# liortalker/MindTheEdge

Hardware: AMD Instinct MI355X
Metric: training images/sec, PackNet-SAN+edge-loss 384x1280 bf16 (higher is better)
Workload: dtype bf16; 1 GPU; T8: PackNet-SAN + silog + 4-scale depth-edge loss training step, 384x1280, 8 frames/GPU, dropout 0.5, flip 0.5; global_batch=8, height=384, width=1280, parallelism=single GPU

## Files before the change

mindtheedge_amd/csrc/heads_misc.hip:

```cpp
#include "common.hpp"
#include <atomic>

int tap_wgrad_mfma_launch(const bf16_t* x, long ldx, const float* m, float* rec, long rec_stride, int B, int H, int W, int C, int sgn, int up2, int has_db,
                          int max_wgs, int* groups, hipStream_t st);
namespace {

template <typename T> __device__ __forceinline__ void ld8(const T* p, float* v);
template <> __device__ __forceinline__ void ld8<bf16_t>(const bf16_t* p, float* v) { unpack16<bf16_t>(*(const u32x4_t*)p, v); }
template <> __device__ __forceinline__ void ld8<float>(const float* p, float* v) {
    unpack16<float>(*(const u32x4_t*)p, v); unpack16<float>(*(const u32x4_t*)(p + 4), v + 4);
}
template <typename T> __device__ __forceinline__ void st8(T* p, const float* v);
template <> __device__ __forceinline__ void st8<bf16_t>(bf16_t* p, const float* v) { *(u32x4_t*)p = pack16<bf16_t>(v); }
template <> __device__ __forceinline__ void st8<float>(float* p, const float* v) {
    *(u32x4_t*)p = pack16<float>(v); *(u32x4_t*)(p + 4) = pack16<float>(v + 4);
}

struct HeadArgs {
    const void* x; long ldx;
    const float* w; const float* bias;
    float* out;
    const float* dlogit;
    void* dx; long lddx;
    float* dw;
// ... 482 lines not shown
#pragma unroll
        for (int r = 0; r < 3; ++r) { const int yy = yl - 1 + r; iok[r] = (unsigned)yy < (unsigned)h; ir[r] = inv + ((long)b * h + min(max(yy, 0), h - 1)) * wl; }
        float uw[3][3];
#pragma unroll
        for (int k = 0; k < 3; ++k) {
            const int xx = x0 - 1 + k; const bool ok = (unsigned)xx < (unsigned)wl; const int xc = min(max(xx, 0), wl - 1);
#pragma unroll
            for (int r = 0; r < 3; ++r) uw[r][k] = (ok && iok[r]) ? ir[r][xc] : 0.f;
        }
        const int x1 = min(x0 + SEG, wl);
        for (int x = x0; x < x1; ++x) {
            u32x4_t raw[4];
#pragma unroll
            for (int q = 0; q < 4; ++q) raw[q] = *(const u32x4_t*)(base + ((long)(q >> 1) * W + 2 * x + (q & 1)) * lddy);
#pragma unroll
            for (int q = 0; q < 4; ++q) {
                float g[P];
                unpack16<T>(raw[q], g);
                const int qy = q >> 1, qx = q & 1;
#pragma unroll
                for (int ky = 0; ky < 3; ++ky)
#pragma unroll
                    for (int kx = 0; kx < 3; ++kx) {
                        const float uu = uw[(qy + ky + 1) >> 1][(qx + kx + 1) >> 1];
#pragma unroll
                        for (int e = 0; e < P; ++e) dacc[ky * 3 + kx][e] = fmaf(g[e], uu, dacc[ky * 3 + kx][e]);
                    }
            }
            if (x + 1 < x1) {
                const int xx = x + 2; const bool ok = xx < wl; const int xc = min(xx, wl - 1);
#pragma unroll
                for (int r = 0; r < 3; ++r) { uw[r][0] = uw[r][1]; uw[r][1] = uw[r][2]; uw[r][2] = (ok && iok[r]) ? ir[r][xc] : 0.f; }
            }
        }
    }
    const int lane = threadIdx.x & 63, wave = threadIdx.x >> 6;
#pragma unroll
    for (int tp = 0; tp < 9; ++tp)
#pragma unroll
        for (int e = 0; e < P; ++e) {
            float v = dacc[tp][e];
            for (int off = cpr; off < 64; off <<= 1) v += __shfl_xor(v, off, 64);
            if (lane < cpr) sred[wave * (N * 9) + (lane * P + e) * 9 + tp] = v;
        }
    __syncthreads();
    for (int i = threadIdx.x; i < N * 9; i += blockDim.x)
        records[(long)blockIdx.x * (N * 9) + i] = (sred[i] + sred[N * 9 + i]) + (sred[2 * N * 9 + i] + sred[3 * N * 9 + i]);
}
__global__ __launch_bounds__(256) void rank1_wgrad_reduce_kernel(const float* __restrict__ records, int nrec, int N, float* __restrict__ dst, long dst_stride) {
    const int i = blockIdx.x * 4 + (threadIdx.x >> 6), lane = threadIdx.x & 63;
    if (i >= N * 9) return;
    float s = 0.f;
    for (int r = lane; r < nrec; r += 64) s += records[(long)r * (N * 9) + i];
    for (int off = 32; off > 0; off >>= 1) s += __shfl_xor(s, off, 64);
    if (lane == 0) dst[(long)(i / 9) * dst_stride + i % 9] = s;
}

__global__ void upsample2_f32_kernel(const float* __restrict__ inv, float* __restrict__ out, int B, int h, int w) {
    const long n = (long)B * 4 * h * w;
    for (long i = blockIdx.x * (long)blockDim.x + threadIdx.x; i < n; i += (long)gridDim.x * blockDim.x) {
        const int X = (int)(i % (2 * w)); const long t = i / (2 * w); const int Y = (int)(t % (2 * h)); const int b = (int)(t / (2 * h));
        out[i] = inv[((long)b * h + (Y >> 1)) * w + (X >> 1)];
    }
}

template <typename T>
__global__ void copy_channels_kernel(const T* __restrict__ src, long lds_, T* __restrict__ dst, long ldd, long npix, int C) {
    constexpr int P = Elem<T>::PER16;
    const int cpr = C / P;
    const long n = npix * cpr;
    for (long i = blockIdx.x * (long)blockDim.x + threadIdx.x; i < n; i += (long)gridDim.x * blockDim.x) {
        const long pix = i / cpr; const int cc = (int)(i % cpr);
        *(u32x4_t*)(dst + pix * ldd + cc * P) = *(const u32x4_t*)(src + pix * lds_ + cc * P);
    }
}

__global__ void split_record_kernel(const float* __restrict__ src, float* __restrict__ d0, int n0, float* __restrict__ d1, int n1) {
    for (int i = blockIdx.x * blockDim.x + threadIdx.x; i < n0 + n1; i += gridDim.x * blockDim.x) {
        const float v = src[i];
        if (i < n0) d0[i] = v; else d1[i - n0] = v;
    }
}

template <typename T>
__global__ void add_channels_kernel(const T* __restrict__ a, long lda, const T* __restrict__ b, long ldb, T* __restrict__ out, long ldo,
                                    long npix, int C) {
    constexpr int P = Elem<T>::PER16;
    const int cpr = C / P;
    const long n = npix * cpr;
    for (long i = blockIdx.x * (long)blockDim.x + threadIdx.x; i < n; i += (long)gridDim.x * blockDim.x) {
        const long pix = i / cpr; const int cc = (int)(i % cpr);
        float va[P], vb[P];
        unpack16<T>(*(const u32x4_t*)(a + pix * lda + cc * P), va);
        unpack16<T>(*(const u32x4_t*)(b + pix * ldb + cc * P), vb);
#pragma unroll
        for (int k = 0; k < P; ++k) va[k] += vb[k];
        *(u32x4_t*)(out + pix * ldo + cc * P) = pack16<T>(va);
    }
}

__global__ void adam_kernel(float* __restrict__ p, const float* __restrict__ g, float* __restrict__ m, float* __restrict__ v,
                            long n, float lr, float b1, float b2, float eps, float bc1, float bc2s, float gscale) {
    const long n4 = n >> 2;
    for (long i = blockIdx.x * (long)blockDim.x + threadIdx.x; i < n4; i += (long)gridDim.x * blockDim.x) {
        f32x4_t pp = ((f32x4_t*)p)[i], gg = ((const f32x4_t*)g)[i], mm = ((f32x4_t*)m)[i], vv = ((f32x4_t*)v)[i];
#pragma unroll
        for (int k = 0; k < 4; ++k) {
            const float gk = gg[k] * gscale;
            mm[k] = b1 * mm[k] + (1.f - b1) * gk;
            vv[k] = b2 * vv[k] + (1.f - b2) * gk * gk;
            const float denom = sqrtf(vv[k]) / bc2s + eps;
            pp[k] -= (lr / bc1) * (mm[k] / denom);
        }
        ((f32x4_t*)p)[i] = pp; ((f32x4_t*)m)[i] = mm; ((f32x4_t*)v)[i] = vv;
    }
    if (blockIdx.x == 0 && threadIdx.x < (n & 3)) {
        const long i = (n4 << 2) + threadIdx.x;
        const float gk = g[i] * gscale;
        const float mk = b1 * m[i] + (1.f - b1) * gk, vk = b2 * v[i] + (1.f - b2) * gk * gk;
        m[i] = mk; v[i] = vk;
        p[i] -= (lr / bc1) * (mk / (sqrtf(vk) / bc2s + eps));
    }
}

__global__ void adam_dev_kernel(float* __restrict__ p, const float* __restrict__ g, float* __restrict__ m, float* __restrict__ v,
                                long n, const float* __restrict__ hyper, float b1, float b2, float eps, float gscale) {
    const float lr = hyper[0], bc1 = hyper[1], bc2s = hyper[2];
    const long n4 = n >> 2;
    for (long i = blockIdx.x * (long)blockDim.x + threadIdx.x; i < n4; i += (long)gridDim.x * blockDim.x) {
        f32x4_t pp = ((f32x4_t*)p)[i], gg = ((const f32x4_t*)g)[i], mm = ((f32x4_t*)m)[i], vv = ((f32x4_t*)v)[i];
#pragma unroll
        for (int k = 0; k < 4; ++k) {
            const float gk = gg[k] * gscale;
            mm[k] = b1 * mm[k] + (1.f - b1) * gk;
            vv[k] = b2 * vv[k] + (1.f - b2) * gk * gk;
            const float denom = sqrtf(vv[k]) / bc2s + eps;
            pp[k] -= (lr / bc1) * (mm[k] / denom);
        }
        ((f32x4_t*)p)[i] = pp; ((f32x4_t*)m)[i] = mm; ((f32x4_t*)v)[i] = vv;
    }
    if (blockIdx.x == 0 && threadIdx.x < (n & 3)) {
        const long i = (n4 << 2) + threadIdx.x;
        const float gk = g[i] * gscale;
        const float mk = b1 * m[i] + (1.f - b1) * gk, vk = b2 * v[i] + (1.f - b2) * gk * gk;
        m[i] = mk; v[i] = vk;
        p[i] -= (lr / bc1) * (mk / (sqrtf(vk) / bc2s + eps));
    }
}

__device__ __forceinline__ void bilin_src(int dst, int in, float scale, int& i0, int& i1, float& l1) {
    float src = scale * ((float)dst + 0.5f) - 0.5f;
    if (src < 0.f) src = 0.f;
    i0 = (int)src; if (i0 > in - 1) i0 = in - 1;
    i1 = i0 < in - 1 ? i0 + 1 : i0;
    l1 = src - (float)i0;
}
__global__ void resize_bilinear_kernel(const float* __restrict__ x, float* __restrict__ y, float* __restrict__ dx, const float* __restrict__ dy,
                                       int B, int h, int w, int H, int W) {
    const float sh = (float)h / (float)H, sw = (float)w / (float)W;
    const long n = (long)B * H * W;
    for (long i = blockIdx.x * (long)blockDim.x + threadIdx.x; i < n; i += (long)gridDim.x * blockDim.x) {
        const int X = (int)(i % W), Y = (int)((i / W) % H), b = (int)(i / ((long)W * H));
        int y0, y1, x0, x1; float ly, lx;
        bilin_src(Y, h, sh, y0, y1, ly); bilin_src(X, w, sw, x0, x1, lx);
        const long base = (long)b * h * w;
        const float w00 = (1.f - ly) * (1.f - lx), w01 = (1.f - ly) * lx, w10 = ly * (1.f - lx), w11 = ly * lx;
        if (y) {
            y[i] = w00 * x[base + (long)y0 * w + x0] + w01 * x[base + (long)y0 * w + x1] + w10 * x[base + (long)y1 * w + x0] + w11 * x[base + (long)y1 * w + x1];
        } else {
            const float g = dy[i];
            atomicAdd(dx + base + (long)y0 * w + x0, w00 * g); atomicAdd(dx + base + (long)y0 * w + x1, w01 * g);
            atomicAdd(dx + base + (long)y1 * w + x0, w10 * g); atomicAdd(dx + base + (long)y1 * w + x1, w11 * g);
        }
    }
}

inline int stream_grid(long n, int per = 256) { long g = (n + per - 1) / per; return (int)(g > 8192 ? 8192 : (g < 1 ? 1 : g)); }
int g_head_mfma = 1;
inline bool head_ok(int C) { const int cb = C >> 3; return C % 8 == 0 && cb >= 1 && cb <= 64 && (cb & (cb - 1)) == 0; }
inline long head_strips(int B, int H, int W, int C) {
    const int pxw = 256 / (C >> 3);
    return (long)((W + pxw - 1) / pxw) * ((H + HEAD_ROWS - 1) / HEAD_ROWS) * B;
}
template <typename F> int head_resident(F f, size_t lds, std::atomic<int>* cache) {
    int v = cache->load(std::memory_order_relaxed);
    if (v == 0) {
        int per_cu = 0, dev = 0, cus = 256;
        if (hipOccupancyMaxActiveBlocksPerMultiprocessor(&per_cu, f, 256, lds) != hipSuccess || per_cu < 1) per_cu = 2;
        hipDeviceProp_t prop;
        if (hipGetDevice(&dev) == hipSuccess && hipGetDeviceProperties(&prop, dev) == hipSuccess && prop.multiProcessorCount > 0) cus = prop.multiProcessorCount;
        v = per_cu * cus;
        cache->store(v, std::memory_order_relaxed);
    }
    return v;
}
inline long head_record_stride(int C) { return ((long)C * 9 + 1 + 3) / 4 * 4; }
constexpr int HEAD_WGRAD_MAX_BLOCKS = 1024;

}

#ifdef MTE_DEV
extern "C" int mtei_set_head_mfma(int v) { g_head_mfma = v; return MTE_OK; }
#endif

extern "C" {

int mte_invdepth_fwd(const void* x, long ldx, const float* w, const float* bias, float* out,
                     int B, int H, int W, int C, float min_depth, int dtype, hipStream_t stream) {
    (void)hipGetLastError();
    if (!x || !w || !bias || !out || !head_ok(C)) return MTE_ERR_ARG;
    HeadArgs a{}; a.x = x; a.ldx = ldx; a.w = w; a.bias = bias; a.out = out; a.B = B; a.H = H; a.W = W; a.C = C;
    a.inv_min_depth = 1.f / min_depth; a.npix = (long)B * H * W;
    if (dtype == MTE_DT_BF16 && g_head_mfma && C % 32 == 0 && C <= ((g_head_mfma & 2) ? 256 : 128) && ldx % 8 == 0) {
        int rows = C >= 128 ? 16 : 32;
        bool pf = C >= 64;
        if (g_head_mfma != 1) {
            pf = (g_head_mfma & 4) != 0;
            if (g_head_mfma >> 8) rows = g_head_mfma >> 8;
        }
        const long g2 = (long)((W + 63) / 64) * ((H + rows - 1) / rows) * B;
        if (g2 <= 0x7fffffffL) {
#define MTE_HEAD_LAUNCH(CS_)                                                                                                              \
            if (pf) hipLaunchKernelGGL((invdepth_fwd_mfma_kernel<CS_, true>), dim3((unsigned)g2), dim3(256), 0, stream, a, rows);       \
            else hipLaunchKernelGGL((invdepth_fwd_mfma_kernel<CS_, false>), dim3((unsigned)g2), dim3(256), 0, stream, a, rows);         \
            return mte_check_launch();
            switch (C / 32) {
                case 1: { MTE_HEAD_LAUNCH(1) }
                case 2: { MTE_HEAD_LAUNCH(2) }
                case 4: { MTE_HEAD_LAUNCH(4) }
                case 8: { MTE_HEAD_LAUNCH(8) }
            }
#undef MTE_HEAD_LAUNCH
        }
    }
    const long grid = head_strips(B, H, W, C);
    if (grid > 0x7fffffffL) return MTE_ERR_UNSUPPORTED;
    if (dtype == MTE_DT_BF16) hipLaunchKernelGGL(invdepth_fwd_kernel<bf16_t>, dim3((unsigned)grid), dim3(256), 0, stream, a);
    else hipLaunchKernelGGL(invdepth_fwd_kernel<float>, dim3((unsigned)grid), dim3(256), 0, stream, a);
    return mte_check_launch();
}

int mte_invdepth_bwd_data(const float* w, const float* inv_out, const float* dout, float* dlogit,
                          void* dx, long lddx, int B, int H, int W, int C, float min_depth, int dtype, hipStream_t stream) {
    (void)hipGetLastError();
    if (!w || !inv_out || !dout || !dlogit || !dx || !head_ok(C)) return MTE_ERR_ARG;
    const long npix = (long)B * H * W;
    hipLaunchKernelGGL(invdepth_dlogit_kernel, dim3(stream_grid(npix)), dim3(256), 0, stream, dout, inv_out, dlogit, npix, 1.f / min_depth);
    HeadArgs a{}; a.w = w; a.dlogit = dlogit; a.dx = dx; a.lddx = lddx; a.B = B; a.H = H; a.W = W; a.C = C; a.npix = npix;
    const long grid = head_strips(B, H, W, C);
    if (grid > 0x7fffffffL) return MTE_ERR_UNSUPPORTED;
    if (dtype == MTE_DT_BF16) hipLaunchKernelGGL(invdepth_bwd_data_kernel<bf16_t>, dim3((unsigned)grid), dim3(256), 0, stream, a);
    else hipLaunchKernelGGL(invdepth_bwd_data_kernel<float>, dim3((unsigned)grid), dim3(256), 0, stream, a);
    return mte_check_launch();
}

long mte_invdepth_bwd_weight_workspace_elems(int C) { return head_ok(C) ? HEAD_WGRAD_MAX_BLOCKS * head_record_stride(C) : 0; }

int mte_invdepth_bwd_weight(const void* x, long ldx, const float* dlogit, float* dwb, float* records,
                            int B, int H, int W, int C, int dtype, hipStream_t stream) {
    (void)hipGetLastError();
// ... 43 lines not shown
}
int mte_upsample_inv_bwd(const void* dsrc, long lds_, float* dinv, int B, int h, int w, int accumulate, int dtype, hipStream_t stream) {
    (void)hipGetLastError();
    if (!dsrc || !dinv) return MTE_ERR_ARG;
    const int grid = stream_grid((long)B * h * w);
    if (dtype == MTE_DT_BF16) hipLaunchKernelGGL(upsample_inv_bwd_kernel<bf16_t>, dim3(grid), dim3(256), 0, stream, (const bf16_t*)dsrc, lds_, dinv, B, h, w, accumulate);
    else hipLaunchKernelGGL(upsample_inv_bwd_kernel<float>, dim3(grid), dim3(256), 0, stream, (const float*)dsrc, lds_, dinv, B, h, w, accumulate);
    return mte_check_launch();
}

int mte_rank1_conv_fwd(const float* inv, const float* w, long w_stride, void* y, long ldy, int B, int h, int wl, int N, int dtype, hipStream_t stream) {
    (void)hipGetLastError();
    if (!inv || !w || !y || N % 32 != 0 || N > 256 || B < 1 || h < 1 || wl < 1) return MTE_ERR_ARG;
    const int per16 = dtype == MTE_DT_BF16 ? 8 : 4;
    const int grid = stream_grid((long)B * 2 * h * ((2 * wl + 63) / 64) * (N / per16));
    if (dtype == MTE_DT_BF16) hipLaunchKernelGGL(rank1_conv_fwd_kernel<bf16_t>, dim3(grid), dim3(256), 0, stream, inv, w, w_stride, (bf16_t*)y, ldy, B, h, wl, N);
    else hipLaunchKernelGGL(rank1_conv_fwd_kernel<float>, dim3(grid), dim3(256), 0, stream, inv, w, w_stride, (float*)y, ldy, B, h, wl, N);
    return mte_check_launch();
}
int mte_rank1_conv_bwd_data(const void* dy, long lddy, const float* w, long w_stride, float* dinv, int B, int h, int wl, int N, int accumulate, int dtype,
                            hipStream_t stream) {
    (void)hipGetLastError();
    if (!dy || !w || !dinv || (N != 32 && N != 64 && N != 128) || B < 1 || h < 1 || wl < 1) return MTE_ERR_ARG;
    const int per16 = dtype == MTE_DT_BF16 ? 8 : 4;
    const int grid = stream_grid((long)B * h * ((wl + 15) / 16) * (N / per16));
    const size_t lds = sizeof(float) * 25 * N;
    if (dtype == MTE_DT_BF16) hipLaunchKernelGGL(rank1_conv_bwd_data_kernel<bf16_t>, dim3(grid), dim3(256), lds, stream, (const bf16_t*)dy, lddy, w, w_stride, dinv, B, h, wl, N, accumulate);
    else hipLaunchKernelGGL(rank1_conv_bwd_data_kernel<float>, dim3(grid), dim3(256), lds, stream, (const float*)dy, lddy, w, w_stride, dinv, B, h, wl, N, accumulate);
    return mte_check_launch();
}
constexpr int RANK1_BWD_WGS = 1024;
long mte_rank1_conv_bwd_records_elems(int N) { return (long)RANK1_BWD_WGS * N * 9; }
int mte_rank1_conv_bwd_weight(const void* dy, long lddy, const float* inv, float* dw, long dw_stride, float* records,
                              int B, int h, int wl, int N, int dtype, hipStream_t stream) {
    (void)hipGetLastError();
    if (!dy || !inv || !dw || !records || (N != 32 && N != 64 && N != 128) || B < 1 || h < 1 || wl < 1) return MTE_ERR_ARG;
    if (dtype == MTE_DT_BF16) {
        int groups = 0;
        const int rc = tap_wgrad_mfma_launch((const bf16_t*)dy, lddy, inv, records, (long)N * 9, B, 2 * h, 2 * wl, N, +1, 1, 0, RANK1_BWD_WGS, &groups, stream);
        if (rc == MTE_OK) {
            hipLaunchKernelGGL(rank1_wgrad_reduce_kernel, dim3((N * 9 + 3) / 4), dim3(256), 0, stream, records, groups, N, dw, dw_stride);
            return mte_check_launch();
        }
        if (rc != MTE_ERR_UNSUPPORTED) return rc;
    }
    const int per16 = dtype == MTE_DT_BF16 ? 8 : 4;
    const long items = (long)B * h * ((wl + 15) / 16) * (N / per16);
    long g = (items + 255) / 256; if (g > RANK1_BWD_WGS) g = RANK1_BWD_WGS; if (g < 1) g = 1;
    const size_t lds = sizeof(float) * 4 * N * 9;
    if (dtype == MTE_DT_BF16) hipLaunchKernelGGL(rank1_conv_bwd_weight_kernel<bf16_t>, dim3((unsigned)g), dim3(256), lds, stream, (const bf16_t*)dy, lddy, inv, records, B, h, wl, N);
    else hipLaunchKernelGGL(rank1_conv_bwd_weight_kernel<float>, dim3((unsigned)g), dim3(256), lds, stream, (const float*)dy, lddy, inv, records, B, h, wl, N);
    hipLaunchKernelGGL(rank1_wgrad_reduce_kernel, dim3((N * 9 + 3) / 4), dim3(256), 0, stream, records, (int)g, N, dw, dw_stride);
    return mte_check_launch();
}
int mte_upsample2_f32(const float* inv, float* out, int B, int h, int wl, hipStream_t stream) {
    (void)hipGetLastError();
    if (!inv || !out || B < 1 || h < 1 || wl < 1) return MTE_ERR_ARG;
    hipLaunchKernelGGL(upsample2_f32_kernel, dim3(stream_grid((long)B * 4 * h * wl)), dim3(256), 0, stream, inv, out, B, h, wl);
    return mte_check_launch();
}

int mte_copy_channels(const void* src, long lds_, void* dst, long ldd, long npix, int C, int dtype, hipStream_t stream) {
    (void)hipGetLastError();
    if (!src || !dst || C % 8 != 0) return MTE_ERR_ARG;
    const int per16 = dtype == MTE_DT_BF16 ? 8 : 4;
    const int grid = stream_grid(npix * (C / per16));
    if (dtype == MTE_DT_BF16) hipLaunchKernelGGL(copy_channels_kernel<bf16_t>, dim3(grid), dim3(256), 0, stream, (const bf16_t*)src, lds_, (bf16_t*)dst, ldd, npix, C);
    else hipLaunchKernelGGL(copy_channels_kernel<float>, dim3(grid), dim3(256), 0, stream, (const float*)src, lds_, (float*)dst, ldd, npix, C);
    return mte_check_launch();
}

int mte_split_record(const float* src, float* dst0, int n0, float* dst1, int n1, hipStream_t stream) {
    (void)hipGetLastError();
    if (!src || !dst0 || !dst1 || n0 < 0 || n1 < 0) return MTE_ERR_ARG;
    if (n0 + n1 == 0) return MTE_OK;
    const int grid = (n0 + n1 + 255) / 256 < 64 ? (n0 + n1 + 255) / 256 : 64;
    hipLaunchKernelGGL(split_record_kernel, dim3(grid), dim3(256), 0, stream, src, dst0, n0, dst1, n1);
    return mte_check_launch();
}

int mte_add_channels(const void* a, long lda, const void* b, long ldb, void* out, long ldo, long npix, int C, int dtype, hipStream_t stream) {
    (void)hipGetLastError();
    const int per16 = dtype == MTE_DT_BF16 ? 8 : 4;
    if (!a || !b || !out || C % per16 != 0) return MTE_ERR_ARG;
    const int grid = stream_grid(npix * (C / per16));
    if (dtype == MTE_DT_BF16) hipLaunchKernelGGL(add_channels_kernel<bf16_t>, dim3(grid), dim3(256), 0, stream, (const bf16_t*)a, lda, (const bf16_t*)b, ldb, (bf16_t*)out, ldo, npix, C);
    else hipLaunchKernelGGL(add_channels_kernel<float>, dim3(grid), dim3(256), 0, stream, (const float*)a, lda, (const float*)b, ldb, (float*)out, ldo, npix, C);
    return mte_check_launch();
}

int mte_adam_step(float* p, const float* g, float* m, float* v, long n, float lr, float beta1, float beta2, float eps,
                  int step, float gscale, hipStream_t stream) {
    (void)hipGetLastError();
    if (!p || !g || !m || !v || n <= 0 || step < 1) return MTE_ERR_ARG;
    const double bc1 = 1.0 - pow((double)beta1, step), bc2 = 1.0 - pow((double)beta2, step);
    hipLaunchKernelGGL(adam_kernel, dim3(stream_grid(n >> 2)), dim3(256), 0, stream, p, g, m, v, n, lr, beta1, beta2, eps,
                       (float)bc1, (float)sqrt(bc2), gscale);
    return mte_check_launch();
}

int mte_resize_bilinear_fwd(const float* x, float* y, int B, int h, int w, int H, int W, hipStream_t stream) {
    (void)hipGetLastError();
    if (!x || !y || B < 1 || h < 1 || w < 1 || H < 1 || W < 1) return MTE_ERR_ARG;
    hipLaunchKernelGGL(resize_bilinear_kernel, dim3(stream_grid((long)B * H * W)), dim3(256), 0, stream, x, y, (float*)nullptr, (const float*)nullptr, B, h, w, H, W);
    return mte_check_launch();
}
int mte_resize_bilinear_bwd(const float* dy, float* dx, int B, int h, int w, int H, int W, hipStream_t stream) {
    (void)hipGetLastError();
    if (!dy || !dx || B < 1 || h < 1 || w < 1 || H < 1 || W < 1) return MTE_ERR_ARG;
    if (mte_memset_async(dx, 0, sizeof(float) * (size_t)B * h * w, stream) != hipSuccess) return MTE_ERR_LAUNCH;
    hipLaunchKernelGGL(resize_bilinear_kernel, dim3(stream_grid((long)B * H * W)), dim3(256), 0, stream, (const float*)nullptr, (float*)nullptr, dx, dy, B, h, w, H, W);
    return mte_check_launch();
}

int mte_adam_step_dev(float* p, const float* g, float* m, float* v, long n, const float* hyper, float beta1, float beta2, float eps,
                      float gscale, hipStream_t stream) {
    (void)hipGetLastError();
    if (!p || !g || !m || !v || !hyper || n <= 0) return MTE_ERR_ARG;
    hipLaunchKernelGGL(adam_dev_kernel, dim3(stream_grid(n >> 2)), dim3(256), 0, stream, p, g, m, v, n, hyper, beta1, beta2, eps, gscale);
    return mte_check_launch();
}

}
```

mindtheedge_amd/csrc/pack_fold.hip:

```cpp
#include "common.hpp"

namespace {

__global__ void fold_weights_kernel(const float* __restrict__ W, const float* __restrict__ K3, const float* __restrict__ b,
                                    const float* __restrict__ b3, float* __restrict__ Wf, float* __restrict__ bf,
                                    int Co, int D, int k) {
    __shared__ float s3[108];
    if (threadIdx.x < 108) s3[threadIdx.x] = K3[threadIdx.x];
    __syncthreads();
    const int K2 = k + 2, kk = k * k;
    const long total = (long)Co * D * K2 * K2;
    for (long i = blockIdx.x * (long)blockDim.x + threadIdx.x; i < total; i += (long)gridDim.x * blockDim.x) {
        const int ux = (int)(i % K2); long t = i / K2;
        const int uy = (int)(t % K2); t /= K2;
        const int c = (int)(t % D); const int co = (int)(t / D);
        float acc = 0.f;
        for (int f = 0; f < 4; ++f)
            for (int kd = 0; kd < 3; ++kd) {
                const int d = c - kd + 1;
                if (d < 0 || d >= D) continue;
                const float* wrow = W + ((long)co * 4 * D + f * D + d) * kk;
#pragma unroll
                for (int dh = 0; dh < 3; ++dh) {
                    const int ty = uy - dh;
// ... 25 lines not shown
        __syncthreads();
        if (lane == 0)
#pragma unroll
            for (int f = 0; f < 4; ++f) s_w[f][wave] = sf[f];
        __syncthreads();
        if (threadIdx.x == 0) {
            float sum = 0.f;
            for (int f = 0; f < 4; ++f) sum = fmaf((s_w[f][0] + s_w[f][1]) + (s_w[f][2] + s_w[f][3]), b3[f], sum);
            bf[co] = b[co] + sum;
        }
    }
}

__global__ void unfold_dw_kernel(const float* __restrict__ dWf, const float* __restrict__ dbf, const float* __restrict__ K3,
                                 const float* __restrict__ b3, float* __restrict__ dW, int Co, int D, int k, int accumulate) {
    __shared__ float s3[108];
    if (threadIdx.x < 108) s3[threadIdx.x] = K3[threadIdx.x];
    __syncthreads();
    const int K2 = k + 2, kk = k * k;
    const long total = (long)Co * 4 * D * kk;
    for (long i = blockIdx.x * (long)blockDim.x + threadIdx.x; i < total; i += (long)gridDim.x * blockDim.x) {
        const int tx = (int)(i % k); long t = i / k;
        const int ty = (int)(t % k); t /= k;
        const int fd = (int)(t % (4 * D)); const int co = (int)(t / (4 * D));
        const int f = fd / D, d = fd - f * D;
        float acc = dbf[co] * b3[f];
        for (int kd = 0; kd < 3; ++kd) {
            const int c = d + kd - 1;
            if (c < 0 || c >= D) continue;
            const float* g = dWf + (((long)co * D + c) * K2) * K2;
#pragma unroll
            for (int dh = 0; dh < 3; ++dh)
#pragma unroll
                for (int dw = 0; dw < 3; ++dw)
                    acc = fmaf(g[(ty + dh) * K2 + tx + dw], s3[((f * 3 + kd) * 3 + dh) * 3 + dw], acc);
        }
        dW[i] = accumulate ? dW[i] + acc : acc;
    }
}

__global__ __launch_bounds__(256) void unfold_dk3_kernel(const float* __restrict__ dWf, const float* __restrict__ dbf,
                                                         const float* __restrict__ W, float* __restrict__ out, int Co, int D, int k) {
    __shared__ float sred[4 * 112];
    const int K2 = k + 2, kk = k * k;
    float acc[112];
#pragma unroll
    for (int i = 0; i < 112; ++i) acc[i] = 0.f;
    const long items = (long)Co * D * kk;
    for (long ix = blockIdx.x * (long)blockDim.x + threadIdx.x; ix < items; ix += (long)gridDim.x * blockDim.x) {
        const int t = (int)(ix % kk); const long rix = ix / kk;
        const int d = (int)(rix % D); const int co = (int)(rix / D);
        const float dbv = dbf[co];
        {
            const int ty = t / k, tx = t - ty * k;
            float wv[4];
#pragma unroll
            for (int f = 0; f < 4; ++f) { wv[f] = W[((long)co * 4 * D + f * D + d) * kk + t]; acc[108 + f] = fmaf(dbv, wv[f], acc[108 + f]); }
#pragma unroll
            for (int kd = 0; kd < 3; ++kd) {
                const int c = d + kd - 1;
                if (c < 0 || c >= D) continue;
                const float* g = dWf + (((long)co * D + c) * K2) * K2;
#pragma unroll
                for (int dh = 0; dh < 3; ++dh)
#pragma unroll
                    for (int dw = 0; dw < 3; ++dw) {
                        const float gv = g[(ty + dh) * K2 + tx + dw];
#pragma unroll
                        for (int f = 0; f < 4; ++f) acc[((f * 3 + kd) * 3 + dh) * 3 + dw] = fmaf(gv, wv[f], acc[((f * 3 + kd) * 3 + dh) * 3 + dw]);
                    }
            }
        }
    }
    const int lane = threadIdx.x & 63, wave = threadIdx.x >> 6;
#pragma unroll
    for (int i = 0; i < 112; ++i) {
        const float s = wave_sum(acc[i]);
        if (lane == 0) sred[wave * 112 + i] = s;
    }
    __syncthreads();
    if (threadIdx.x < 112) atomicAdd(out + threadIdx.x, sred[threadIdx.x] + sred[112 + threadIdx.x] + sred[224 + threadIdx.x] + sred[336 + threadIdx.x]);
}

template <typename T>
__global__ void pixel_shuffle_kernel(const T* __restrict__ src, long lds_, T* __restrict__ dst, long ldd, int B, int H, int W, int C, int dir) {
    const int H2 = H >> 1, W2 = W >> 1, cb = C >> 3;
    const long total = (long)B * H2 * W2 * cb;
    for (long i = blockIdx.x * (long)blockDim.x + threadIdx.x; i < total; i += (long)gridDim.x * blockDim.x) {
        const int j = (int)(i % cb); long t = i / cb;
        const int w = (int)(t % W2); t /= W2;
        const int h = (int)(t % H2); const int b = (int)(t / H2);
        float v[4][8];
        if (dir == 0) {
#pragma unroll
            for (int s = 0; s < 4; ++s) {
                const T* p = src + (((long)b * H + 2 * h + (s >> 1)) * W + 2 * w + (s & 1)) * lds_ + j * 8;
                if constexpr (sizeof(T) == 2) unpack16<bf16_t>(*(const u32x4_t*)p, v[s]);
                else { unpack16<float>(*(const u32x4_t*)p, v[s]); unpack16<float>(*(const u32x4_t*)(p + 4), v[s] + 4); }
            }
            T* q = dst + (((long)b * H2 + h) * W2 + w) * ldd + 32 * j;
#pragma unroll
            for (int k8 = 0; k8 < 4; ++k8) {
                float o[8];
#pragma unroll
                for (int e = 0; e < 8; ++e) o[e] = v[e & 3][2 * k8 + (e >> 2)];
                if constexpr (sizeof(T) == 2) *(u32x4_t*)(q + 8 * k8) = pack16<bf16_t>(o);
                else { *(u32x4_t*)(q + 8 * k8) = pack16<float>(o); *(u32x4_t*)(q + 8 * k8 + 4) = pack16<float>(o + 4); }
            }
        } else {
            const T* q = src + (((long)b * H2 + h) * W2 + w) * lds_ + 32 * j;
            float o[4][8];
#pragma unroll
            for (int k8 = 0; k8 < 4; ++k8) {
                if constexpr (sizeof(T) == 2) unpack16<bf16_t>(*(const u32x4_t*)(q + 8 * k8), o[k8]);
                else { unpack16<float>(*(const u32x4_t*)(q + 8 * k8), o[k8]); unpack16<float>(*(const u32x4_t*)(q + 8 * k8 + 4), o[k8] + 4); }
            }
#pragma unroll
            for (int s = 0; s < 4; ++s) {
                float xv[8];
#pragma unroll
                for (int c = 0; c < 8; ++c) xv[c] = o[c >> 1][(c & 1) * 4 + s];
                T* p = dst + (((long)b * H + 2 * h + (s >> 1)) * W + 2 * w + (s & 1)) * ldd + j * 8;
                if constexpr (sizeof(T) == 2) *(u32x4_t*)p = pack16<bf16_t>(xv);
                else { *(u32x4_t*)p = pack16<float>(xv); *(u32x4_t*)(p + 4) = pack16<float>(xv + 4); }
            }
        }
    }
}

template <typename T>
__global__ void copy_rect_kernel(const T* __restrict__ src, long lds_, int Hs, int Ws, int sy, int sx,
                                 T* __restrict__ dst, long ldd, int Hd, int Wd, int dy, int dx, int B, int h, int w, int C, int mode) {
    constexpr int P = Elem<T>::PER16;
    const int cpr = C / P;
    const long total = (long)B * h * w * cpr;
    for (long i = blockIdx.x * (long)blockDim.x + threadIdx.x; i < total; i += (long)gridDim.x * blockDim.x) {
        const int cc = (int)(i % cpr); long t = i / cpr;
        const int x = (int)(t % w); t /= w;
        const int y = (int)(t % h); const int b = (int)(t / h);
        T* q = dst + (((long)b * Hd + dy + y) * Wd + dx + x) * ldd + cc * P;
        if (mode == 2) { *(u32x4_t*)q = u32x4_t{0u, 0u, 0u, 0u}; continue; }
        const u32x4_t sv = *(const u32x4_t*)(src + (((long)b * Hs + sy + y) * Ws + sx + x) * lds_ + cc * P);
        if (mode == 0) *(u32x4_t*)q = sv;
        else {
            float a[P], c[P];
            unpack16<T>(sv, a); unpack16<T>(*(const u32x4_t*)q, c);
#pragma unroll
            for (int e = 0; e < P; ++e) c[e] += a[e];
            *(u32x4_t*)q = pack16<T>(c);
        }
    }
}

struct RectOp { const void* src; long lds_; int Hs, Ws, sy, sx; void* dst; long ldd; int Hd, Wd, dy, dx, h, w, mode; };
struct RectOps { RectOp op[8]; };

template <typename T>
__global__ void copy_rects_kernel(RectOps ops, int B, int C) {
    const RectOp& o = ops.op[blockIdx.y];
    constexpr int P = Elem<T>::PER16;
    const int cpr = C / P;
    const long total = (long)B * o.h * o.w * cpr;
    const T* src = (const T*)o.src;
    T* dst = (T*)o.dst;
    for (long i = blockIdx.x * (long)blockDim.x + threadIdx.x; i < total; i += (long)gridDim.x * blockDim.x) {
        const int cc = (int)(i % cpr); long t = i / cpr;
        const int x = (int)(t % o.w); t /= o.w;
        const int y = (int)(t % o.h); const int b = (int)(t / o.h);
        T* q = dst + (((long)b * o.Hd + o.dy + y) * o.Wd + o.dx + x) * o.ldd + cc * P;
        if (o.mode == 2) { *(u32x4_t*)q = u32x4_t{0u, 0u, 0u, 0u}; continue; }
        const u32x4_t sv = *(const u32x4_t*)(src + (((long)b * o.Hs + o.sy + y) * o.Ws + o.sx + x) * o.lds_ + cc * P);
        if (o.mode == 0) *(u32x4_t*)q = sv;
        else {
            float a[P], c[P];
            unpack16<T>(sv, a); unpack16<T>(*(const u32x4_t*)q, c);
#pragma unroll
            for (int e = 0; e < P; ++e) c[e] += a[e];
            *(u32x4_t*)q = pack16<T>(c);
        }
    }
}

inline int sgrid(long n) { long g = (n + 255) / 256; return (int)(g > 8192 ? 8192 : (g < 1 ? 1 : g)); }

}

extern "C" {

int mte_fold_pack_weights(const float* W, const float* K3, const float* b, const float* b3, float* Wf, float* bf,
                          int Co, int D, int k, hipStream_t stream) {
    (void)hipGetLastError();
    if (!W || !K3 || !b || !b3 || !Wf || !bf || (k & 1) == 0) return MTE_ERR_ARG;
    hipLaunchKernelGGL(fold_weights_kernel, dim3(sgrid((long)Co * D * (k + 2) * (k + 2))), dim3(256), 0, stream, W, K3, b, b3, Wf, bf, Co, D, k);
    return mte_check_launch();
}

int mte_unfold_pack_wgrad(const float* dWf, const float* dbf, const float* W, const float* K3, const float* b3,
                          float* dW, float* dk3b, int Co, int D, int k, int accumulate, hipStream_t stream) {
    (void)hipGetLastError();
    if (!dWf || !dbf || !W || !K3 || !b3 || !dW || !dk3b) return MTE_ERR_ARG;
    hipLaunchKernelGGL(unfold_dw_kernel, dim3(sgrid((long)Co * 4 * D * k * k)), dim3(256), 0, stream, dWf, dbf, K3, b3, dW, Co, D, k, accumulate);
    long items = (long)Co * D * k * k;
    long g = (items + 255) / 256; if (g > 512) g = 512; if (g < 1) g = 1;
    hipLaunchKernelGGL(unfold_dk3_kernel, dim3((unsigned)g), dim3(256), 0, stream, dWf, dbf, W, dk3b, Co, D, k);
    return mte_check_launch();
}

int mte_pixel_shuffle(const void* src, long lds_, void* dst, long ldd, int B, int H, int W, int C, int dir, int dtype, hipStream_t stream) {
    (void)hipGetLastError();
    if (!src || !dst || C % 8 != 0 || (H & 1) || (W & 1)) return MTE_ERR_ARG;
    const int grid = sgrid((long)B * (H / 2) * (W / 2) * (C / 8));
    if (dtype == MTE_DT_BF16) hipLaunchKernelGGL(pixel_shuffle_kernel<bf16_t>, dim3(grid), dim3(256), 0, stream, (const bf16_t*)src, lds_, (bf16_t*)dst, ldd, B, H, W, C, dir);
    else hipLaunchKernelGGL(pixel_shuffle_kernel<float>, dim3(grid), dim3(256), 0, stream, (const float*)src, lds_, (float*)dst, ldd, B, H, W, C, dir);
    return mte_check_launch();
}

int mte_copy_rect(const void* src, long lds_, int Hs, int Ws, int sy, int sx, void* dst, long ldd, int Hd, int Wd, int dy, int dx,
                  int B, int h, int w, int C, int mode, int dtype, hipStream_t stream) {
    (void)hipGetLastError();
    if (!dst || (mode != 2 && !src) || C % 8 != 0 || h <= 0 || w <= 0) return MTE_ERR_ARG;
    if (sy < 0 || sx < 0 || dy < 0 || dx < 0 || dy + h > Hd || dx + w > Wd || (mode != 2 && (sy + h > Hs || sx + w > Ws))) return MTE_ERR_ARG;
    const int per16 = dtype == MTE_DT_BF16 ? 8 : 4;
    const int grid = sgrid((long)B * h * w * (C / per16));
    if (dtype == MTE_DT_BF16) hipLaunchKernelGGL(copy_rect_kernel<bf16_t>, dim3(grid), dim3(256), 0, stream, (const bf16_t*)src, lds_, Hs, Ws, sy, sx, (bf16_t*)dst, ldd, Hd, Wd, dy, dx, B, h, w, C, mode);
    else hipLaunchKernelGGL(copy_rect_kernel<float>, dim3(grid), dim3(256), 0, stream, (const float*)src, lds_, Hs, Ws, sy, sx, (float*)dst, ldd, Hd, Wd, dy, dx, B, h, w, C, mode);
    return mte_check_launch();
}

int mte_copy_rects(const void* ops_host, int n, int B, int C, int dtype, hipStream_t stream) {
    (void)hipGetLastError();
    if (!ops_host || n < 1 || n > 8 || C % 8 != 0) return MTE_ERR_ARG;
    RectOps ops{};
    long most = 0;
    const int per16 = dtype == MTE_DT_BF16 ? 8 : 4;
    for (int i = 0; i < n; ++i) {
        const RectOp& o = ((const RectOp*)ops_host)[i];
        if (!o.dst || (o.mode != 2 && !o.src) || o.h <= 0 || o.w <= 0) return MTE_ERR_ARG;
        if (o.sy < 0 || o.sx < 0 || o.dy < 0 || o.dx < 0 || o.dy + o.h > o.Hd || o.dx + o.w > o.Wd ||
            (o.mode != 2 && (o.sy + o.h > o.Hs || o.sx + o.w > o.Ws))) return MTE_ERR_ARG;
        ops.op[i] = o;
        const long t = (long)B * o.h * o.w * (C / per16);
        if (t > most) most = t;
    }
    const dim3 grid(sgrid(most), n);
    if (dtype == MTE_DT_BF16) hipLaunchKernelGGL(copy_rects_kernel<bf16_t>, grid, dim3(256), 0, stream, ops, B, C);
    else hipLaunchKernelGGL(copy_rects_kernel<float>, grid, dim3(256), 0, stream, ops, B, C);
    return mte_check_launch();
}

}
```

Baseline: 374.7 images/sec.

## Rework streaming copy/add/pixel-shuffle kernels with incremental indexing and batched loads

Rewrites the add_channels, pixel_shuffle and copy_rect(s) kernels to use 32-bit incremental mixed-radix index stepping instead of per-iteration 64-bit div/mod. Loads are grouped ahead of stores (depth-2 for rects) to keep more memory requests in flight. The grid is sized to whole CU rounds rather than capped at 8192 blocks. Pixel shuffle gets compile-time direction and bf16 register-level packing so it no longer round-trips through float. This targets the address-arithmetic and latency overhead of these bandwidth-bound helpers, but adds 32-bit item-count limits and a hardcoded 256-CU assumption.

```diff
diff --git a/mindtheedge_amd/csrc/heads_misc.hip b/mindtheedge_amd/csrc/heads_misc.hip
--- a/mindtheedge_amd/csrc/heads_misc.hip
+++ b/mindtheedge_amd/csrc/heads_misc.hip
@@ -588,20 +588,43 @@
     }
 }
 
-template <typename T>
-__global__ void add_channels_kernel(const T* __restrict__ a, long lda, const T* __restrict__ b, long ldb, T* __restrict__ out, long ldo,
-                                    long npix, int C) {
+#ifndef MTE_ADD_DEPTH
+#define MTE_ADD_DEPTH 1
+#endif
+#ifndef MTE_STREAM_WG_PER_CU
+#define MTE_STREAM_WG_PER_CU 64
+#endif
+constexpr int ADD_DEPTH = MTE_ADD_DEPTH;
+template <typename T>
+__global__ __launch_bounds__(256) void add_channels_kernel(const T* a, long lda, const T* __restrict__ b, long ldb, T* out, long ldo, unsigned n, int cpr) {
     constexpr int P = Elem<T>::PER16;
-    const int cpr = C / P;
-    const long n = npix * cpr;
-    for (long i = blockIdx.x * (long)blockDim.x + threadIdx.x; i < n; i += (long)gridDim.x * blockDim.x) {
-        const long pix = i / cpr; const int cc = (int)(i % cpr);
-        float va[P], vb[P];
-        unpack16<T>(*(const u32x4_t*)(a + pix * lda + cc * P), va);
-        unpack16<T>(*(const u32x4_t*)(b + pix * ldb + cc * P), vb);
-#pragma unroll
-        for (int k = 0; k < P; ++k) va[k] += vb[k];
-        *(u32x4_t*)(out + pix * ldo + cc * P) = pack16<T>(va);
+    const unsigned S = gridDim.x * 256u;
+    const unsigned spix = S / (unsigned)cpr; const int scc = (int)(S - spix * (unsigned)cpr);
+    unsigned i = blockIdx.x * 256u + threadIdx.x;
+    unsigned pix = i / (unsigned)cpr; int cc = (int)(i - pix * (unsigned)cpr);
+    for (; i < n; i += ADD_DEPTH * S) {
+        u32x4_t ca[ADD_DEPTH], cb[ADD_DEPTH];
+        T* q[ADD_DEPTH];
+#pragma unroll
+        for (int u = 0; u < ADD_DEPTH; ++u) {
+            if (i + u * S < n) {
+                ca[u] = *(const u32x4_t*)(a + (long)pix * lda + cc * P);
+                cb[u] = *(const u32x4_t*)(b + (long)pix * ldb + cc * P);
+                q[u] = out + (long)pix * ldo + cc * P;
+            }
+            cc += scc; const int c = cc >= cpr; cc -= c ? cpr : 0;
+            pix += spix + c;
+        }
+#pragma unroll
+        for (int u = 0; u < ADD_DEPTH; ++u) {
+            if (i + u * S < n) {
+                float va[P], vb[P];
+                unpack16<T>(ca[u], va); unpack16<T>(cb[u], vb);
+#pragma unroll
+                for (int k = 0; k < P; ++k) va[k] += vb[k];
+                *(u32x4_t*)q[u] = pack16<T>(va);
+            }
+        }
     }
 }
 
@@ -682,6 +705,13 @@
 }
 
 inline int stream_grid(long n, int per = 256) { long g = (n + per - 1) / per; return (int)(g > 8192 ? 8192 : (g < 1 ? 1 : g)); }
+inline int stream_rounds(long items, int per_wg) {
+    constexpr long CUS = 256, ONE_TRIP = CUS * MTE_STREAM_WG_PER_CU;
+    const long need = (items + per_wg - 1) / per_wg;
+    if (need <= ONE_TRIP) return (int)(need < 1 ? 1 : need);
+    const long trips = (need + ONE_TRIP - 1) / ONE_TRIP;
+    return (int)(((need + trips - 1) / trips + CUS - 1) / CUS * CUS);
+}
 int g_head_mfma = 1;
 inline bool head_ok(int C) { const int cb = C >> 3; return C % 8 == 0 && cb >= 1 && cb <= 64 && (cb & (cb - 1)) == 0; }
 inline long head_strips(int B, int H, int W, int C) {
@@ -891,10 +921,14 @@
 int mte_add_channels(const void* a, long lda, const void* b, long ldb, void* out, long ldo, long npix, int C, int dtype, hipStream_t stream) {
     (void)hipGetLastError();
     const int per16 = dtype == MTE_DT_BF16 ? 8 : 4;
-    if (!a || !b || !out || C % per16 != 0) return MTE_ERR_ARG;
-    const int grid = stream_grid(npix * (C / per16));
-    if (dtype == MTE_DT_BF16) hipLaunchKernelGGL(add_channels_kernel<bf16_t>, dim3(grid), dim3(256), 0, stream, (const bf16_t*)a, lda, (const bf16_t*)b, ldb, (bf16_t*)out, ldo, npix, C);
-    else hipLaunchKernelGGL(add_channels_kernel<float>, dim3(grid), dim3(256), 0, stream, (const float*)a, lda, (const float*)b, ldb, (float*)out, ldo, npix, C);
+    if (!a || !b || !out || C % per16 != 0 || C < 0 || npix < 0) return MTE_ERR_ARG;
+    const int cpr = C / per16;
+    if (cpr > 0 && npix > 0x7fffffffL / cpr) return MTE_ERR_ARG;
+    const long n = npix * cpr;
+    if (n == 0) return MTE_OK;
+    const dim3 grid(stream_rounds(n, 256 * ADD_DEPTH));
+    if (dtype == MTE_DT_BF16) hipLaunchKernelGGL(add_channels_kernel<bf16_t>, grid, dim3(256), 0, stream, (const bf16_t*)a, lda, (const bf16_t*)b, ldb, (bf16_t*)out, ldo, (unsigned)n, cpr);
+    else hipLaunchKernelGGL(add_channels_kernel<float>, grid, dim3(256), 0, stream, (const float*)a, lda, (const float*)b, ldb, (float*)out, ldo, (unsigned)n, cpr);
     return mte_check_launch();
 }
 
diff --git a/mindtheedge_amd/csrc/pack_fold.hip b/mindtheedge_amd/csrc/pack_fold.hip
--- a/mindtheedge_amd/csrc/pack_fold.hip
+++ b/mindtheedge_amd/csrc/pack_fold.hip
@@ -131,104 +131,170 @@
     if (threadIdx.x < 112) atomicAdd(out + threadIdx.x, sred[threadIdx.x] + sred[112 + threadIdx.x] + sred[224 + threadIdx.x] + sred[336 + threadIdx.x]);
 }
 
+#ifndef MTE_PS_DEPTH
+#define MTE_PS_DEPTH 1
+#endif
+#ifndef MTE_STREAM_WG_PER_CU
+#define MTE_STREAM_WG_PER_CU 64
+#endif
+constexpr int PS_DEPTH = MTE_PS_DEPTH;
+constexpr int STREAM_CUS = 256;
+constexpr int STREAM_ONE_TRIP = STREAM_CUS * MTE_STREAM_WG_PER_CU;
+
+struct Radix { int n0, n1, n2; };
+struct Digits { int d0, d1, d2, d3; };
+__device__ __forceinline__ Digits split_item(unsigned i, const Radix& r) {
+    Digits d;
+    unsigned t = i / (unsigned)r.n0; d.d0 = (int)(i - t * (unsigned)r.n0);
+    unsigned u = t / (unsigned)r.n1; d.d1 = (int)(t - u * (unsigned)r.n1);
+    t = u / (unsigned)r.n2; d.d2 = (int)(u - t * (unsigned)r.n2);
+    d.d3 = (int)t;
+    return d;
+}
+__device__ __forceinline__ void step_item(Digits& d, const Digits& s, const Radix& r) {
+    d.d0 += s.d0; int c = d.d0 >= r.n0; d.d0 -= c ? r.n0 : 0;
+    d.d1 += s.d1 + c; c = d.d1 >= r.n1; d.d1 -= c ? r.n1 : 0;
+    d.d2 += s.d2 + c; c = d.d2 >= r.n2; d.d2 -= c ? r.n2 : 0;
+    d.d3 += s.d3 + c;
+}
+
+inline int stream_rounds(long items, int per_wg) {
+    const long need = (items + per_wg - 1) / per_wg;
+    if (need <= STREAM_ONE_TRIP) return (int)(need < 1 ? 1 : need);
+    const long trips = (need + STREAM_ONE_TRIP - 1) / STREAM_ONE_TRIP;
+    const long g = ((need + trips - 1) / trips + STREAM_CUS - 1) / STREAM_CUS * STREAM_CUS;
+    return (int)g;
+}
+
+__device__ __forceinline__ unsigned lo2(unsigned a, unsigned b) { return (a & 0xffffu) | (b << 16); }
+__device__ __forceinline__ unsigned hi2(unsigned a, unsigned b) { return (a >> 16) | (b & 0xffff0000u); }
+
+template <int NV> __device__ __forceinline__ void ps_pack(const u32x4_t (&xr)[4][NV], u32x4_t (&pr)[4][NV]) {
+#pragma unroll
+    for (int k = 0; k < 4; ++k) {
+        if constexpr (NV == 1) {
+            pr[k][0] = u32x4_t{lo2(xr[0][0][k], xr[1][0][k]), lo2(xr[2][0][k], xr[3][0][k]), hi2(xr[0][0][k], xr[1][0][k]), hi2(xr[2][0][k], xr[3][0][k])};
+        } else {
+#pragma unroll
+            for (int e = 0; e < 2; ++e) {
+                const int c = 2 * k + e;
+                pr[k][e] = u32x4_t{xr[0][c >> 2][c & 3], xr[1][c >> 2][c & 3], xr[2][c >> 2][c & 3], xr[3][c >> 2][c & 3]};
+            }
+        }
+    }
+}
+template <int NV> __device__ __forceinline__ void ps_unpack(const u32x4_t (&pr)[4][NV], u32x4_t (&xr)[4][NV]) {
+#pragma unroll
+    for (int s = 0; s < 4; ++s) {
+        if constexpr (NV == 1) {
+#pragma unroll
+            for (int i = 0; i < 4; ++i) {
+                const unsigned a = pr[i][0][s >> 1], b = pr[i][0][2 + (s >> 1)];
+                xr[s][0][i] = (s & 1) ? hi2(a, b) : lo2(a, b);
+            }
+        } else {
+#pragma unroll
+            for (int c = 0; c < 8; ++c) xr[s][c >> 2][c & 3] = pr[c >> 1][c & 1][s];
+        }
+    }
+}
+
+template <typename T, int DIR>
+__global__ __launch_bounds__(256) void pixel_shuffle_kernel(const T* __restrict__ src, long lds_, T* __restrict__ dst, long ldd, int H2, int W, int cb, unsigned items) {
+    constexpr int P = Elem<T>::PER16, NV = 8 / P;
+    const Radix r{cb, W >> 1, H2};
+    const unsigned S = gridDim.x * 256u;
+    const Digits sd = split_item(S, r);
+    unsigned i = blockIdx.x * 256u + threadIdx.x;
+    Digits d = split_item(i, r);
+    const long ldx = DIR == 0 ? lds_ : ldd, ldp = DIR == 0 ? ldd : lds_;
+    for (; i < items; i += PS_DEPTH * S) {
+        u32x4_t v[PS_DEPTH][4][NV];
+        long xo[PS_DEPTH], po[PS_DEPTH];
+#pragma unroll
+        for (int u = 0; u < PS_DEPTH; ++u) {
+            if (i + u * S < items) {
+                const long row = (long)d.d3 * H2 + d.d2;
+                xo[u] = (2 * row * W + 2 * d.d1) * ldx + 8 * d.d0;
+                po[u] = (row * (W >> 1) + d.d1) * ldp + 32 * d.d0;
+#pragma unroll
+                for (int s = 0; s < 4; ++s)
+#pragma unroll
+                    for (int e = 0; e < NV; ++e)
+                        v[u][s][e] = DIR == 0 ? *(const u32x4_t*)(src + xo[u] + ((long)(s >> 1) * W + (s & 1)) * ldx + e * P)
+                                              : *(const u32x4_t*)(src + po[u] + (s * NV + e) * P);
+            }
+            step_item(d, sd, r);
+        }
+#pragma unroll
+        for (int u = 0; u < PS_DEPTH; ++u) {
+            if (i + u * S < items) {
+                u32x4_t o[4][NV];
+                if constexpr (DIR == 0) ps_pack<NV>(v[u], o); else ps_unpack<NV>(v[u], o);
+#pragma unroll
+                for (int s = 0; s < 4; ++s)
+#pragma unroll
+                    for (int e = 0; e < NV; ++e) {
+                        if constexpr (DIR == 0) *(u32x4_t*)(dst + po[u] + (s * NV + e) * P) = o[s][e];
+                        else *(u32x4_t*)(dst + xo[u] + ((long)(s >> 1) * W + (s & 1)) * ldx + e * P) = o[s][e];
+                    }
+            }
+        }
+    }
+}
+
+struct RectOp { const void* src; long lds_; int Hs, Ws, sy, sx; void* dst; long ldd; int Hd, Wd, dy, dx, h, w, mode; };
+
 template <typename T>
-__global__ void pixel_shuffle_kernel(const T* __restrict__ src, long lds_, T* __restrict__ dst, long ldd, int B, int H, int W, int C, int dir) {
-    const int H2 = H >> 1, W2 = W >> 1, cb = C >> 3;
-    const long total = (long)B * H2 * W2 * cb;
-    for (long i = blockIdx.x * (long)blockDim.x + threadIdx.x; i < total; i += (long)gridDim.x * blockDim.x) {
-        const int j = (int)(i % cb); long t = i / cb;
-        const int w = (int)(t % W2); t /= W2;
-        const int h = (int)(t % H2); const int b = (int)(t / H2);
-        float v[4][8];
-        if (dir == 0) {
-#pragma unroll
-            for (int s = 0; s < 4; ++s) {
-                const T* p = src + (((long)b * H + 2 * h + (s >> 1)) * W + 2 * w + (s & 1)) * lds_ + j * 8;
-                if constexpr (sizeof(T) == 2) unpack16<bf16_t>(*(const u32x4_t*)p, v[s]);
-                else { unpack16<float>(*(const u32x4_t*)p, v[s]); unpack16<float>(*(const u32x4_t*)(p + 4), v[s] + 4); }
-            }
-            T* q = dst + (((long)b * H2 + h) * W2 + w) * ldd + 32 * j;
-#pragma unroll
-            for (int k8 = 0; k8 < 4; ++k8) {
-                float o[8];
-#pragma unroll
-                for (int e = 0; e < 8; ++e) o[e] = v[e & 3][2 * k8 + (e >> 2)];
-                if constexpr (sizeof(T) == 2) *(u32x4_t*)(q + 8 * k8) = pack16<bf16_t>(o);
-                else { *(u32x4_t*)(q + 8 * k8) = pack16<float>(o); *(u32x4_t*)(q + 8 * k8 + 4) = pack16<float>(o + 4); }
-            }
-        } else {
-            const T* q = src + (((long)b * H2 + h) * W2 + w) * lds_ + 32 * j;
-            float o[4][8];
-#pragma unroll
-            for (int k8 = 0; k8 < 4; ++k8) {
-                if constexpr (sizeof(T) == 2) unpack16<bf16_t>(*(const u32x4_t*)(q + 8 * k8), o[k8]);
-                else { unpack16<float>(*(const u32x4_t*)(q + 8 * k8), o[k8]); unpack16<float>(*(const u32x4_t*)(q + 8 * k8 + 4), o[k8] + 4); }
-            }
-#pragma unroll
-            for (int s = 0; s < 4; ++s) {
-                float xv[8];
-#pragma unroll
-                for (int c = 0; c < 8; ++c) xv[c] = o[c >> 1][(c & 1) * 4 + s];
-                T* p = dst + (((long)b * H + 2 * h + (s >> 1)) * W + 2 * w + (s & 1)) * ldd + j * 8;
-                if constexpr (sizeof(T) == 2) *(u32x4_t*)p = pack16<bf16_t>(xv);
-                else { *(u32x4_t*)p = pack16<float>(xv); *(u32x4_t*)(p + 4) = pack16<float>(xv + 4); }
-            }
-        }
-    }
-}
-
-template <typename T>
-__global__ void copy_rect_kernel(const T* __restrict__ src, long lds_, int Hs, int Ws, int sy, int sx,
-                                 T* __restrict__ dst, long ldd, int Hd, int Wd, int dy, int dx, int B, int h, int w, int C, int mode) {
+__device__ __forceinline__ void rect_op(const RectOp& o, int B, int C) {
     constexpr int P = Elem<T>::PER16;
-    const int cpr = C / P;
-    const long total = (long)B * h * w * cpr;
-    for (long i = blockIdx.x * (long)blockDim.x + threadIdx.x; i < total; i += (long)gridDim.x * blockDim.x) {
-        const int cc = (int)(i % cpr); long t = i / cpr;
-        const int x = (int)(t % w); t /= w;
-        const int y = (int)(t % h); const int b = (int)(t / h);
-        T* q = dst + (((long)b * Hd + dy + y) * Wd + dx + x) * ldd + cc * P;
-        if (mode == 2) { *(u32x4_t*)q = u32x4_t{0u, 0u, 0u, 0u}; continue; }
-        const u32x4_t sv = *(const u32x4_t*)(src + (((long)b * Hs + sy + y) * Ws + sx + x) * lds_ + cc * P);
-        if (mode == 0) *(u32x4_t*)q = sv;
-        else {
-            float a[P], c[P];
-            unpack16<T>(sv, a); unpack16<T>(*(const u32x4_t*)q, c);
-#pragma unroll
-            for (int e = 0; e < P; ++e) c[e] += a[e];
-            *(u32x4_t*)q = pack16<T>(c);
-        }
-    }
-}
-
-struct RectOp { const void* src; long lds_; int Hs, Ws, sy, sx; void* dst; long ldd; int Hd, Wd, dy, dx, h, w, mode; };
-struct RectOps { RectOp op[8]; };
-
-template <typename T>
-__global__ void copy_rects_kernel(RectOps ops, int B, int C) {
-    const RectOp& o = ops.op[blockIdx.y];
-    constexpr int P = Elem<T>::PER16;
-    const int cpr = C / P;
-    const long total = (long)B * o.h * o.w * cpr;
+    const Radix r{C / P, o.w, o.h};
+    const unsigned items = (unsigned)B * o.h * o.w * r.n0;
+    const unsigned S = gridDim.x * 256u;
+    unsigned i = blockIdx.x * 256u + threadIdx.x;
+    if (i >= items) return;
+    const Digits sd = split_item(S, r);
+    Digits d = split_item(i, r);
     const T* src = (const T*)o.src;
     T* dst = (T*)o.dst;
-    for (long i = blockIdx.x * (long)blockDim.x + threadIdx.x; i < total; i += (long)gridDim.x * blockDim.x) {
-        const int cc = (int)(i % cpr); long t = i / cpr;
-        const int x = (int)(t % o.w); t /= o.w;
-        const int y = (int)(t % o.h); const int b = (int)(t / o.h);
-        T* q = dst + (((long)b * o.Hd + o.dy + y) * o.Wd + o.dx + x) * o.ldd + cc * P;
-        if (o.mode == 2) { *(u32x4_t*)q = u32x4_t{0u, 0u, 0u, 0u}; continue; }
-        const u32x4_t sv = *(const u32x4_t*)(src + (((long)b * o.Hs + o.sy + y) * o.Ws + o.sx + x) * o.lds_ + cc * P);
-        if (o.mode == 0) *(u32x4_t*)q = sv;
-        else {
-            float a[P], c[P];
-            unpack16<T>(sv, a); unpack16<T>(*(const u32x4_t*)q, c);
-#pragma unroll
-            for (int e = 0; e < P; ++e) c[e] += a[e];
-            *(u32x4_t*)q = pack16<T>(c);
-        }
-    }
-}
+    for (; i < items; i += 2 * S) {
+        T* q[2];
+        u32x4_t sv[2], dv[2];
+#pragma unroll
+        for (int u = 0; u < 2; ++u) {
+            if (i + u * S < items) {
+                q[u] = dst + (((long)d.d3 * o.Hd + o.dy + d.d2) * o.Wd + o.dx + d.d1) * o.ldd + d.d0 * P;
+                if (o.mode != 2) sv[u] = *(const u32x4_t*)(src + (((long)d.d3 * o.Hs + o.sy + d.d2) * o.Ws + o.sx + d.d1) * o.lds_ + d.d0 * P);
+                if (o.mode == 1) dv[u] = *(const u32x4_t*)q[u];
+            }
+            step_item(d, sd, r);
+        }
+#pragma unroll
+        for (int u = 0; u < 2; ++u) {
+            if (i + u * S < items) {
+                if (o.mode == 2) *(u32x4_t*)q[u] = u32x4_t{0u, 0u, 0u, 0u};
+                else if (o.mode == 0) *(u32x4_t*)q[u] = sv[u];
+                else {
+                    float a[P], c[P];
+                    unpack16<T>(sv[u], a); unpack16<T>(dv[u], c);
+#pragma unroll
+                    for (int e = 0; e < P; ++e) c[e] += a[e];
+                    *(u32x4_t*)q[u] = pack16<T>(c);
+                }
+            }
+        }
+    }
+}
+
+template <typename T>
+__global__ __launch_bounds__(256) void copy_rect_kernel(RectOp op, int B, int C) { rect_op<T>(op, B, C); }
+
+struct RectOps { RectOp op[8]; };
+
+template <typename T>
+__global__ __launch_bounds__(256) void copy_rects_kernel(RectOps ops, int B, int C) { rect_op<T>(ops.op[blockIdx.y], B, C); }
+
+inline int rect_grid(long items) { return items <= (long)STREAM_ONE_TRIP * 256 ? stream_rounds(items, 256) : stream_rounds(items, 512); }
 
 inline int sgrid(long n) { long g = (n + 255) / 256; return (int)(g > 8192 ? 8192 : (g < 1 ? 1 : g)); }
 
@@ -257,10 +323,20 @@
 
 int mte_pixel_shuffle(const void* src, long lds_, void* dst, long ldd, int B, int H, int W, int C, int dir, int dtype, hipStream_t stream) {
     (void)hipGetLastError();
-    if (!src || !dst || C % 8 != 0 || (H & 1) || (W & 1)) return MTE_ERR_ARG;
-    const int grid = sgrid((long)B * (H / 2) * (W / 2) * (C / 8));
-    if (dtype == MTE_DT_BF16) hipLaunchKernelGGL(pixel_shuffle_kernel<bf16_t>, dim3(grid), dim3(256), 0, stream, (const bf16_t*)src, lds_, (bf16_t*)dst, ldd, B, H, W, C, dir);
-    else hipLaunchKernelGGL(pixel_shuffle_kernel<float>, dim3(grid), dim3(256), 0, stream, (const float*)src, lds_, (float*)dst, ldd, B, H, W, C, dir);
+    if (!src || !dst || C % 8 != 0 || (H & 1) || (W & 1) || B < 0 || H < 0 || W < 0 || C < 0) return MTE_ERR_ARG;
+    const long items = (long)B * (H / 2) * (W / 2) * (C / 8);
+    if (items > 0x7fffffffL) return MTE_ERR_ARG;
+    if (items == 0) return MTE_OK;
+    const dim3 grid(stream_rounds(items, 256 * PS_DEPTH));
+    const int H2 = H / 2, cb = C / 8;
+    const unsigned n = (unsigned)items;
+    if (dtype == MTE_DT_BF16) {
+        if (dir == 0) hipLaunchKernelGGL((pixel_shuffle_kernel<bf16_t, 0>), grid, dim3(256), 0, stream, (const bf16_t*)src, lds_, (bf16_t*)dst, ldd, H2, W, cb, n);
+        else hipLaunchKernelGGL((pixel_shuffle_kernel<bf16_t, 1>), grid, dim3(256), 0, stream, (const bf16_t*)src, lds_, (bf16_t*)dst, ldd, H2, W, cb, n);
+    } else {
+        if (dir == 0) hipLaunchKernelGGL((pixel_shuffle_kernel<float, 0>), grid, dim3(256), 0, stream, (const float*)src, lds_, (float*)dst, ldd, H2, W, cb, n);
+        else hipLaunchKernelGGL((pixel_shuffle_kernel<float, 1>), grid, dim3(256), 0, stream, (const float*)src, lds_, (float*)dst, ldd, H2, W, cb, n);
+    }
     return mte_check_launch();
 }
 
@@ -269,16 +345,20 @@
     (void)hipGetLastError();
     if (!dst || (mode != 2 && !src) || C % 8 != 0 || h <= 0 || w <= 0) return MTE_ERR_ARG;
     if (sy < 0 || sx < 0 || dy < 0 || dx < 0 || dy + h > Hd || dx + w > Wd || (mode != 2 && (sy + h > Hs || sx + w > Ws))) return MTE_ERR_ARG;
-    const int per16 = dtype == MTE_DT_BF16 ? 8 : 4;
-    const int grid = sgrid((long)B * h * w * (C / per16));
-    if (dtype == MTE_DT_BF16) hipLaunchKernelGGL(copy_rect_kernel<bf16_t>, dim3(grid), dim3(256), 0, stream, (const bf16_t*)src, lds_, Hs, Ws, sy, sx, (bf16_t*)dst, ldd, Hd, Wd, dy, dx, B, h, w, C, mode);
-    else hipLaunchKernelGGL(copy_rect_kernel<float>, dim3(grid), dim3(256), 0, stream, (const float*)src, lds_, Hs, Ws, sy, sx, (float*)dst, ldd, Hd, Wd, dy, dx, B, h, w, C, mode);
+    if (B < 0 || C < 0) return MTE_ERR_ARG;
+    const long items = (long)B * h * w * (C / (dtype == MTE_DT_BF16 ? 8 : 4));
+    if (items > 0x7fffffffL) return MTE_ERR_ARG;
+    if (items == 0) return MTE_OK;
+    const RectOp op{src, lds_, Hs, Ws, sy, sx, dst, ldd, Hd, Wd, dy, dx, h, w, mode};
+    const dim3 grid(rect_grid(items));
+    if (dtype == MTE_DT_BF16) hipLaunchKernelGGL(copy_rect_kernel<bf16_t>, grid, dim3(256), 0, stream, op, B, C);
+    else hipLaunchKernelGGL(copy_rect_kernel<float>, grid, dim3(256), 0, stream, op, B, C);
     return mte_check_launch();
 }
 
 int mte_copy_rects(const void* ops_host, int n, int B, int C, int dtype, hipStream_t stream) {
     (void)hipGetLastError();
-    if (!ops_host || n < 1 || n > 8 || C % 8 != 0) return MTE_ERR_ARG;
+    if (!ops_host || n < 1 || n > 8 || C % 8 != 0 || B < 0 || C < 0) return MTE_ERR_ARG;
     RectOps ops{};
     long most = 0;
     const int per16 = dtype == MTE_DT_BF16 ? 8 : 4;
@@ -291,7 +371,9 @@
         const long t = (long)B * o.h * o.w * (C / per16);
         if (t > most) most = t;
     }
-    const dim3 grid(sgrid(most), n);
+    if (most > 0x7fffffffL) return MTE_ERR_ARG;
+    if (most == 0) return MTE_OK;
+    const dim3 grid(rect_grid(most), n);
     if (dtype == MTE_DT_BF16) hipLaunchKernelGGL(copy_rects_kernel<bf16_t>, grid, dim3(256), 0, stream, ops, B, C);
     else hipLaunchKernelGGL(copy_rects_kernel<float>, grid, dim3(256), 0, stream, ops, B, C);
     return mte_check_launch();
```

Result: no change. 375.5 images/sec (median of 6 runs) (+0.2%).
